# Nikhil-AI-Labs/image-super-resolution-2

Measured on AMD Instinct MI355X. Metric: output MPix/s at x4 SR (256->1024), higher is better.
Workload: dtype bf16 (bf16 MFMA operands, fp32 accumulate, fp32 activations in HBM); 1 GPU; FreqFusion x4 full 3-expert forward (HAT-L + DAT + NAFNet-SR + fusion stack), one 256x256 LR tile -> 1024x1024 per step per GPU (BASELINE configs[1]); seeded synthetic weights (172.3 M params), 1/f-noise tiles; tile=256, parallelism=tile-sharded x1, weights RCCL-broadcast once (0.0 ms), no per-tile collectives, launch=hipGraph replay, tiles_in_flight=2

## Files before the change

### image-super-resolution-2_amd/build.py

```python
from __future__ import annotations

import os
import subprocess
import sys
from concurrent.futures import ThreadPoolExecutor

HERE = os.path.dirname(os.path.abspath(__file__))
CSRC = os.path.join(HERE, "csrc")
LIB = os.path.join(HERE, "libff_hip.so")
SOURCES = ["ff_runtime.hip", "conv_gemm.hip", "conv_gemm_bf16.hip", "gemm_rows_bf16.hip", "conv3x3_halo.hip", "sgfn_tail.hip", "ocab_attn.hip", "conv3x3_small.hip", "attention.hip", "attention_bf16.hip", "win_attn_fused.hip", "hab_link.hip", "chan_qkv.hip", "token_mlp.hip", "token_linear.hip", "naf_fused.hip", "naf_tail.hip", "norm_pool.hip", "dwconv.hip", "elementwise.hip",
           "resample.hip", "freq.hip", "fusion_ops.hip", "metrics.hip", "train_ops.hip", "sr_losses.hip", "augment.hip", "ff_executor.hip"]
HIPCC = os.environ.get("HIPCC", "/opt/rocm/bin/hipcc")
FLAGS = ["--offload-arch=gfx950", "-O3", "-fPIC", "-std=c++17", "-Wall", "-Wno-unused-function", "-I" + os.path.join(HERE, "build")]


def _stale() -> bool:
    if not os.path.exists(LIB):
        return True
    t = os.path.getmtime(LIB)
    deps = [os.path.join(CSRC, f) for f in os.listdir(CSRC)] + [os.path.join(HERE, "..", "include", "ff_kernels.h")]
    return any(os.path.getmtime(d) > t for d in deps)


def gen_dispatch(path: str) -> None:
    from .lib import parse_header
    protos = {n: p for n, p in parse_header().items() if p[1] and p[1][-1] == "void*" and p[0] == "int"
              and n not in ("ff_forward", "ff_create", "ff_upload")}
    names = sorted(protos)
    out = ["// generated by build.py from include/ff_kernels.h -- do not edit", f"#define FF_DISPATCH_COUNT {len(names)}",
           "static const char* const FF_DISPATCH_NAMES[FF_DISPATCH_COUNT] = {" + ", ".join(f'"{n}"' for n in names) + "};"]
    def kinds(n):
        ks = []
        for i, ty in enumerate(protos[n][1]):
# ... 57 lines not shown
```

### image-super-resolution-2_amd/csrc/conv3x3_halo.hip

```cpp
#include "ff_common.h"

struct HaloParams {
  const float* in; const unsigned char* w; const float* bias; const float* mul; const float* res; float* out;
  int B, H, W, Cin, ldi, Cout, ldo, ldr, nchunk, tiles_x, tiles_y, nblk, act, shuffle;
  float alpha;
  float* pool_part;
  int vec_epi;
  int io_bf16;
  int images;
  FF_STAMP_MEMBER
};

#define HX_ROW 272
#define HX_W 18
#define HX_PROW 5120

template <int N> __device__ __forceinline__ void halo_wait_vmcnt() {
  static_assert(N >= 0 && N <= 12, "counted vmcnt out of range");
  if constexpr (N == 0) asm volatile("s_waitcnt vmcnt(0)" ::: "memory");
  else if constexpr (N == 1) asm volatile("s_waitcnt vmcnt(1)" ::: "memory");
  else if constexpr (N == 2) asm volatile("s_waitcnt vmcnt(2)" ::: "memory");
  else if constexpr (N == 3) asm volatile("s_waitcnt vmcnt(3)" ::: "memory");
  else if constexpr (N == 4) asm volatile("s_waitcnt vmcnt(4)" ::: "memory");
  else if constexpr (N == 5) asm volatile("s_waitcnt vmcnt(5)" ::: "memory");
// ... 206 lines not shown
            }
  #pragma unroll
            for (int i = 0; i < MI; ++i)
  #pragma unroll
              for (int j = 0; j < NI; ++j) {
                if (NTERMS == 3) {
                  acc[i][j] = __builtin_amdgcn_mfma_f32_32x32x16_bf16(ah[i], bl[j], acc[i][j], 0, 0, 0);
                  acc[i][j] = __builtin_amdgcn_mfma_f32_32x32x16_bf16(al[i], bh[j], acc[i][j], 0, 0, 0);
                }
                acc[i][j] = __builtin_amdgcn_mfma_f32_32x32x16_bf16(ah[i], bh[j], acc[i][j], 0, 0, 0);
              }
          }
        }
      }
      if (chunk + 1 < p.nchunk) {
        __syncthreads();
        if (!XPREF) load_x(chunk + 1);
        store_x();
      }
    }
  }
  FF_STAMP(8, 2);
  if (p.vec_epi) {
    asm volatile("s_waitcnt lgkmcnt(0)" ::: "memory");
    __builtin_amdgcn_s_barrier();
    float* ps = reinterpret_cast<float*>(smem);
    float* patch = reinterpret_cast<float*>(smem + 8192) + wid * (32 * 36);
    const int tq = lane >> 3, q4 = 4 * (lane & 7);
    const bool has_res = p.res != nullptr;
    constexpr bool RES_AHEAD = !(TWO_PER_CU || (NTERMS == 1 && MI * NI <= 2 && WM * WN == 4));
    f32x4 rq[2][MI][4];
    auto load_res = [&](int j, f32x4 (&dst)[MI][4]) {
#pragma unroll
      for (int i = 0; i < MI; ++i)
#pragma unroll
        for (int k = 0; k < 4; ++k) {
          const int mrow = tq + 8 * k, c4 = n0 + wc * TN + j * 32 + q4;
          const int oy = y0 + (wr * MI + i) * 2 + (mrow >> 4), ox = x0 + (mrow & 15);
          const bool ok = c4 < p.Cout && oy < p.H && ox < p.W;
          dst[i][k] = ok ? *reinterpret_cast<const f32x4*>(p.res + ((long long)(b * p.H + oy) * p.W + ox) * p.ldr + c4) : (f32x4){0.f, 0.f, 0.f, 0.f};
        }
    };
    if (RES_AHEAD && has_res) load_res(0, rq[0]);
#pragma unroll
    for (int j = 0; j < NI; ++j) {
      const int n = n0 + wc * TN + j * 32 + l31;
      const bool nok = n < p.Cout;
      const float bv = (nok && p.bias) ? p.bias[n] : 0.f;
      const float mv = ((nok && p.mul) ? p.mul[n] : 1.f) * p.alpha;
      const int c4 = n0 + wc * TN + j * 32 + q4;
      const bool cok = c4 < p.Cout;
      if (RES_AHEAD && has_res && j + 1 < NI) load_res(j + 1, rq[(j + 1) & 1]);
      f32x4 mv4 = {p.alpha, p.alpha, p.alpha, p.alpha};
      if (p.mul && cok) mv4 = *reinterpret_cast<const f32x4*>(p.mul + c4) * p.alpha;
      float psum = 0.f;
#pragma unroll
      for (int i = 0; i < MI; ++i) {
        const int ry0 = y0 + (wr * MI + i) * 2;
#pragma unroll
        for (int r = 0; r < 16; ++r) {
          const int mrow = (r & 3) + 8 * (r >> 2) + 4 * hh;
          const float a = ff_act_c<ACT, true>(acc[i][j][r] + bv);
          patch[mrow * 36 + l31] = a;
          if (nok && ry0 + (mrow >> 4) < p.H && x0 + (mrow & 15) < p.W) psum += a * mv;
        }
#pragma unroll
        for (int k = 0; k < 4; ++k) {
          const int mrow = tq + 8 * k;
          const int oy = ry0 + (mrow >> 4), ox = x0 + (mrow & 15);
          const bool ok = cok && oy < p.H && ox < p.W;
          const f32x4 a4 = *reinterpret_cast<const f32x4*>(patch + mrow * 36 + q4);
          const long long pix = ok ? ((long long)(b * p.H + oy) * p.W + ox) : 0;
          f32x4 r4 = {0.f, 0.f, 0.f, 0.f};
          if (RES_AHEAD && has_res) r4 = rq[j & 1][i][k];
          else if (has_res && ok) r4 = *reinterpret_cast<const f32x4*>(p.res + pix * p.ldr + c4);
          f32x4 v4;
#pragma unroll
          for (int e = 0; e < 4; ++e) v4[e] = __builtin_fmaf(a4[e], mv4[e], r4[e]);
          if (ok) {
            if (NTERMS == 1 && (p.io_bf16 & 2)) {
              bf16x4 h4;
#pragma unroll
              for (int e = 0; e < 4; ++e) h4[e] = (__bf16)v4[e];
              *reinterpret_cast<bf16x4*>(reinterpret_cast<__bf16*>(p.out) + pix * p.ldo + c4) = h4;
            } else {
              *reinterpret_cast<f32x4*>(p.out + pix * p.ldo + c4) = v4;
            }
          }
        }
      }
      if (p.pool_part) {
        psum += __shfl_xor(psum, 32);
        if (hh == 0) ps[wr * BN + wc * TN + j * 32 + l31] = psum;
      }
    }
    if (p.pool_part) {
      __syncthreads();
      for (int c = threadIdx.x; c < BN; c += NT) {
        float sacc = 0.f;
#pragma unroll
        for (int w = 0; w < WM; ++w) sacc += ps[w * BN + c];
        p.pool_part[(long long)blockIdx.x * BN + c] = sacc;
      }
    }
  } else
  {
    const bool has_res = p.res != nullptr;
#pragma unroll
    for (int j = 0; j < NI; ++j) {
      const int n = n0 + wc * TN + j * 32 + l31;
      const bool nok = n < p.Cout;
      const int nc = nok ? n : 0;
      const float bv = (nok && p.bias) ? p.bias[n] : 0.f;
      const float mv = ((nok && p.mul) ? p.mul[n] : 1.f) * p.alpha;
      float psum = 0.f;
#pragma unroll
      for (int i = 0; i < MI; ++i) {
        long long oidx[16];
        float rv[16];
        bool okp[16];
        const int ry0 = y0 + (wr * MI + i) * 2;
#pragma unroll
        for (int r = 0; r < 16; ++r) {
          const int mrow = (r & 3) + 8 * (r >> 2) + 4 * hh;
          const int oy = ry0 + (mrow >> 4), ox = x0 + (mrow & 15);
          okp[r] = nok && oy < p.H && ox < p.W;
          if (p.shuffle == 2) {
// ... 161 lines not shown
```

### image-super-resolution-2_amd/experts.py

```python
from __future__ import annotations

from typing import Dict, List, Optional

import torch

from . import ops
from .prep import (pack_conv, pack_dw, bn_scale_shift, fold_bn_after_conv, pack_token_linear, pack_naf_ffn, pack_naf_tail,
                   pack_win_attn, pack_win_rel, pack_token_projmlp, pack_chan_qkv, pack_token_linear_gated, pack_rel_overlap, pack_ocab_qkv)

T = torch.Tensor
SD = Dict[str, T]
RGB_MEAN = (0.4488, 0.4371, 0.4040)


def _ceil_to(n: int, m: int) -> int:
    return (n + m - 1) // m * m


class _Weights:

    def __init__(self, sd: SD, dev, prefix: str):
        self.sd, self.dev, self.p = sd, dev, prefix

    def __call__(self, name: str) -> T:
# ... 116 lines not shown
            self.gconv.append((w.conv(f"layers.{g}.conv"), w(f"layers.{g}.conv.bias")))

    def _mlp(self, x: T, blk: dict) -> T:
        xn = ops.layernorm(x, *blk["n2"])
        h = ops.linear(xn, *blk["fc1"], act="gelu")
        return ops.linear(h, *blk["fc2"], res=x)

    def hab(self, x: T, blk: dict) -> T:
        _, H, W, C = x.shape
        d = C // self.heads
        fused = ops.fused_modes()
        b16 = ops.gemm_mode() == "bf16" and H * W >= 1024 and C % 4 == 0
        att = ops.empty_rows_bf16(tuple(x.shape), x.device) if b16 else ops.empty_like_rows(x)
        s = blk["shift"]
        if fused:
            relp = _packed(blk, "relp", lambda: pack_win_rel(blk["rel"], self.ws, self.ws))
            _, xn = ops.win_attn_fused(x, att, _wf(blk, self.heads, d), relp, gamma=blk["n1"][0], beta=blk["n1"][1], H=H, W=W,
                                       Hp=H, Wp=W, win=(self.ws, self.ws), shift=(s, s), use_mask=s > 0, want_xn="bf16" if b16 else True)
        else:
            xn = ops.layernorm(x, *blk["n1"])
            qkv = ops.linear(xn, *blk["qkv"])
            ops.window_attn(qkv, att, blk["bias"], q_off=0, k_off=C, v_off=2 * C, o_off=0, H=H, W=W, Hp=H, Wp=W, win=(self.ws, self.ws),
                            kwin=(self.ws, self.ws), shift=(s, s), use_mask=s > 0, heads=self.heads, d=d, scale=d ** -0.5)
        c1 = ops.conv2d(xn, *blk["cab0"], ksize=(3, 3), pad=(1, 1), act="gelu", out_bf16=b16, per_image=True)
        c2, c2mean = ops.conv2d(c1, *blk["cab2"], ksize=(3, 3), pad=(1, 1), want_pool="partials", out_bf16=b16)
        gate = ops.vec_mlp(c2mean, *blk["ca1"], "relu", *blk["ca2"], "sigmoid", post=self.conv_scale)
        if fused:
            return ops.token_projmlp(att, x, _pm(blk), blk["n2"][0], blk["n2"][1], c2=c2, c2_scale=gate if x.shape[0] > 1 else gate.reshape(-1))
        t = ops.mix2(x, c2, cb=gate)
        x = ops.linear(att, *blk["proj"], res=t)
        return self._mlp(x, blk)

    def ocab_block(self, x: T, blk: dict) -> T:
        _, H, W, C = x.shape
        d = C // self.heads
        fused = ops.fused_modes()
        rows16 = ops.gemm_mode() == "bf16" and (self.ws, self.ows, d) == (16, 24, 30) and H % 16 == 0 and W % 16 == 0
        if rows16:
            pk = _packed(blk, "qkv_r16", lambda: pack_ocab_qkv(*blk["qkv"], self.heads, d))
            qkv = ops.token_linear_rows16(x, pk, gamma=blk["n1"][0], beta=blk["n1"][1])
        elif fused:
            qkv = ops.token_linear(x, _tl(blk, "qkv"), gamma=blk["n1"][0], beta=blk["n1"][1])
        else:
            qkv = ops.linear(ops.layernorm(x, *blk["n1"]), *blk["qkv"])
        if rows16:
            att = ops.empty_rows_bf16(tuple(x.shape), x.device)
            hp = self.heads * 32
            ops.ocab_attn_rows16(qkv, att, blk["rel"], q_off=0, k_off=hp, v_off=2 * hp, H=H, W=W, heads=self.heads, d=d, ws=self.ws,
                                 ows=self.ows)
        else:
            att = ops.empty_like_rows(x)
            ops.window_attn(qkv, att, blk["bias"], q_off=0, k_off=C, v_off=2 * C, o_off=0, H=H, W=W, Hp=H, Wp=W, win=(self.ws, self.ws),
                            kwin=(self.ows, self.ows), shift=(0, 0), use_mask=False, heads=self.heads, d=d, scale=d ** -0.5)
        if fused:
            return ops.token_projmlp(att, x, _pm(blk), blk["n2"][0], blk["n2"][1])
        x = ops.linear(att, *blk["proj"], res=x)
        return self._mlp(x, blk)

    def _linked(self, x: T) -> bool:
        B, H, W, C = x.shape
        return (ops.gemm_mode() == "bf16" and H * W >= 1024 and (self.ws, self.heads, C) == (16, 6, 180) and H % 16 == 0 and W % 16 == 0
                and B * H * W * 192 < 2 ** 31)

    def _habs_linked(self, x: T, blks: List[dict]) -> T:
        B, H, W, C = x.shape
        d, win = C // self.heads, (self.ws, self.ws)

        def relp(blk):
            return _packed(blk, "relp", lambda: pack_win_rel(blk["rel"], self.ws, self.ws))

        s = blks[0]["shift"]
        att = ops.empty_rows_bf16(tuple(x.shape), x.device)
        _, xn = ops.win_attn_fused(x, att, _wf(blks[0], self.heads, d), relp(blks[0]), gamma=blks[0]["n1"][0], beta=blks[0]["n1"][1], H=H, W=W,
                                   Hp=H, Wp=W, win=win, shift=(s, s), use_mask=s > 0, want_xn="bf16")
        for i, blk in enumerate(blks):
            c1 = ops.conv2d(xn, *blk["cab0"], ksize=(3, 3), pad=(1, 1), act="gelu", out_bf16=True, per_image=True)
            c2, c2mean = ops.conv2d(c1, *blk["cab2"], ksize=(3, 3), pad=(1, 1), want_pool="partials", out_bf16=True)
            gate = ops.vec_mlp(c2mean, *blk["ca1"], "relu", *blk["ca2"], "sigmoid", post=self.conv_scale)
            gate = gate if B > 1 else gate.reshape(-1)
            if i + 1 < len(blks):
                nxt = blks[i + 1]
                s = nxt["shift"]
                x, xn, att = ops.hab_link(att, x, _pm(blk), blk["n2"][0], blk["n2"][1], c2=c2, c2_scale=gate, wf=_wf(nxt, self.heads, d),
                                          rel_padded=relp(nxt), gamma1=nxt["n1"][0], beta1=nxt["n1"][1], shift=(s, s), use_mask=s > 0)
            else:
                x = ops.token_projmlp(att, x, _pm(blk), blk["n2"][0], blk["n2"][1], c2=c2, c2_scale=gate)
        return x

    def group(self, x: T, g: int) -> T:
        if self._linked(x):
            y = self._habs_linked(x, self.blocks[g])
        else:
            y = x
            for blk in self.blocks[g]:
                y = self.hab(y, blk)
        y = self.ocab_block(y, self.ocab[g])
        return ops.conv2d(y, *self.gconv[g], ksize=(3, 3), pad=(1, 1), res=x, per_image=True)

    def forward(self, lr: T, taps: Optional[dict] = None, feats: Optional[dict] = None, out: Optional[T] = None) -> T:
        B, _, h, w = lr.shape
# ... 351 lines not shown
```

### image-super-resolution-2_amd/ops.py

```python
from __future__ import annotations

from typing import Dict, Optional, Tuple

import torch

from . import lib as _lib

ACT = {None: 0, "none": 0, "gelu": 1, "relu": 2, "lrelu": 3, "sigmoid": 4}
T = torch.Tensor

_PROF = None
_META = [0.0, 0.0]


def _note(flops: float = 0.0, nbytes: float = 0.0):
    _META[0] += flops
    _META[1] += nbytes


def _numel(*ts) -> float:
    return float(sum(t.numel() * (t.element_size() / 4.0) for t in ts if t is not None))


def _instrument(fn):
# ... 686 lines not shown
    if tuple(c2_scale.shape) not in (((K,), (1, K)) if B == 1 else ((B, K),)) or not c2_scale.is_contiguous():
        raise _lib.FFError(f"hab_link: c2_scale must be [{K}] for one image or one row per image [{B},{K}], got {tuple(c2_scale.shape)}")
    if tuple(rel_padded.shape[:2]) != (wf["heads"], 31) or not rel_padded.is_contiguous():
        raise _lib.FFError("hab_link: rel_padded must be [heads][31][stride]")
    out = empty_like_rows(x)
    op_, ldo_, *_ = _nhwc(out, "hab_link.out")
    xn = empty_rows_bf16(tuple(x.shape), x.device)
    xnp, ldxn, *_ = _nhwc(xn, "hab_link.xn|bf16ok")
    ao = empty_rows_bf16(tuple(x.shape), x.device)
    aop, ldao, *_ = _nhwc(ao, "hab_link.att_out|bf16ok")
    m = pk["mlp"]
    _lib.check(_L().ff_hab_link(ap, lda, xp, ldx, cp, ldc, _ptr(c2_scale), K, B, H * W, op_, ldo_, B * H * W, K, m["ht"],
                                pk["proj"]["w"].data_ptr(), pk["proj"]["b"].data_ptr(), gamma2.data_ptr(), beta2.data_ptr(), float(eps2),
                                m["w"].data_ptr(), m["b1"].data_ptr(), m["b2"].data_ptr(), 1, 3,
                                aop, ldao, 0, gamma1.data_ptr(), beta1.data_ptr(), float(eps1), wf["w"].data_ptr(), wf["b"].data_ptr(),
                                rel_padded.data_ptr(), rel_padded.shape[1], rel_padded.shape[2], H, W, 16, 16, shift[0], shift[1],
                                int(use_mask), wf["heads"], wf["d"], xnp, ldxn, 1, 1, _stream()))
    rows, nwin, nh, d = B * H * W, B * (H // 16) * (W // 16), wf["heads"], wf["d"]
    _note(2.0 * rows * K * K + 4.0 * rows * K * m["ht"] * 32 + 2.0 * nwin * 256 * K * 3 * nh * d + 4.0 * nwin * nh * 256 * 256 * d,
          4.0 * rows * K * 3.0 + 4.0 * rows * (K * 0.5 + nh * d * 0.5))
    return out, xn, ao


def token_linear(x: T, pk: dict, *, gamma: Optional[T] = None, beta: Optional[T] = None, eps: float = 1e-5, act=None,
                 res: Optional[T] = None, res2: Optional[T] = None, res2_scale: Optional[T] = None, want_xn: bool = False,
                 stats_range: Optional[Tuple[int, int]] = None, stats_eps: float = 1e-5):
    xp, ldx, rows, K = rows_view(x, "token_linear.x")
    if K != pk["K"]:
        raise _lib.FFError("token_linear: K mismatch")
    N = pk["N"]
    out = empty_rows(tuple(x.shape[:-1]) + (N,), x.device)
    op, ldo, _, _ = rows_view(out, "token_linear.out")
    rp, ldr, r2p, ldr2 = None, 0, None, 0
    if res is not None:
        rp, ldr, rr, rc = rows_view(res, "token_linear.res")
        if rr != rows or rc != N:
            raise _lib.FFError("token_linear: res shape mismatch")
    if res2 is not None:
        r2p, ldr2, rr, rc = rows_view(res2, "token_linear.res2")
        if rr != rows or rc != N or res2_scale is None or res2_scale.numel() != N:
            raise _lib.FFError("token_linear: res2 shape mismatch")
    xn, xnp, ldxn = None, None, 0
    if want_xn:
        if gamma is None:
            raise _lib.FFError("token_linear: want_xn needs LayerNorm parameters")
        xn = empty_like_rows(x)
# ... 778 lines not shown
            _AA_TABLES.clear()
        span, wt = aa_tables(n_in, n_out)
        ent = _AA_TABLES[key] = (torch.from_numpy(span).to(device), torch.from_numpy(wt).to(device))
    return ent


def resize_aa(x: T, size: Tuple[int, int]) -> T:
    _chk(x, "resize_aa.x")
    if x.dim() != 4 or x.shape[1] != 3 or not x.is_contiguous() or x.numel() == 0:
        raise _lib.FFError("resize_aa: expected a non-empty contiguous [B,3,H,W] tensor")
    B, C, Hi, Wi = x.shape
    Ho, Wo = (int(v) for v in size)
    if Ho < 1 or Wo < 1 or Hi != 4 * Ho or Wi != 4 * Wo:
        raise _lib.FFError(f"resize_aa: only the x1/4 ratio is built: {Hi}x{Wi} -> {Ho}x{Wo} is refused")
    span_w, wt_w = _aa_tables_dev(Wi, Wo, x.device)
    span_h, wt_h = _aa_tables_dev(Hi, Ho, x.device)
    out = torch.empty((B, C, Ho, Wo), device=x.device, dtype=torch.float32)
    _lib.check(_L().ff_resize_aa(x.data_ptr(), out.data_ptr(), B * C, Hi, Wi, Ho, Wo, span_w.data_ptr(), wt_w.data_ptr(),
                                 span_h.data_ptr(), wt_h.data_ptr(), _stream()))
    _note(0.0, 4.0 * B * C * (Hi * Wi + Ho * Wo))
    return out


for _n in ("conv2d", "sgfn_tail", "ocab_attn", "ocab_attn_rows16", "token_linear_rows16", "linear", "win_attn_fused", "token_projmlp", "hab_link", "token_linear_gated", "token_mlp", "token_linear", "pixel_mlp", "dwconv3_gate_pool", "naf_front", "naf_ffn", "naf_tail", "window_attn", "layernorm", "pool_mean", "vec_mlp", "dwconv2d", "dwconv3x3_ln", "mix2", "fma3", "affine",
           "nchw_to_nhwc", "nhwc_to_nchw", "resize", "avgpool2", "dct8_bands", "dwt_pass", "fft_bands", "chan_attn_weights", "chan_qkv_attn",
           "band_mha_core", "band_weight", "freq_guidance", "dynamic_gates", "fuse_blend", "tile_accum", "tile_normalize"):
    globals()[_n] = _instrument(globals()[_n])
```

### include/ff_kernels.h

```cpp
#ifndef FF_KERNELS_H
#define FF_KERNELS_H
#ifdef __cplusplus
extern "C" {
#endif

#define FF_ACT_NONE 0
#define FF_ACT_GELU 1
#define FF_ACT_RELU 2
#define FF_ACT_LRELU 3
#define FF_ACT_SIGMOID 4

const char* ff_last_error(void);
int ff_abi_version(void);
int ff_device_cu_count(void);

int ff_conv2d(const float* in, const float* w, const float* bias, const float* mul, const float* res, float* out,
              int B, int H, int W, int Cin, int ldi, int Ho, int Wo, int Cout, int ldo, int ldr, int KH, int KW,
              int sy, int sx, int py, int px, int act, float alpha, int shuffle, int tile_hint, void* stream);

int ff_conv2d_bf16s(const float* in, const void* w_hi, const void* w_lo, int Kp, int Cp, const float* bias, const float* mul,
                    const float* res, float* out, int B, int H, int W, int Cin, int ldi, int Ho, int Wo, int Cout,
                    int ldo, int ldr, int KH, int KW, int sy, int sx, int py, int px, int act, float alpha, int shuffle,
                    int nterms, int tile_hint, const float* kmul, void* stream);
int ff_conv2d_bf16s_tile(long long M, int Cout, int K, int vec4);
// ... 46 lines not shown
int ff_hab_link(const float* att, int lda, const float* x, int ldx, const float* c2, int ldc, const float* c2_scale,
                int scale_ld, int B, long long rows_per_image, float* x_out, int ldxo, long long M, int K, int hidden_tiles,
                const void* proj_tiles, const float* proj_bias_padded, const float* gamma2, const float* beta2, float eps2,
                const void* mlp_tiles, const float* b1_padded, const float* b2, int nterms, int io_bf16,
                float* att_out, int ldo, int o_off, const float* gamma1, const float* beta1, float eps1,
                const void* qkv_tiles, const float* qkv_bias_padded, const float* rel_padded, int rel_rows, int rel_stride,
                int H, int W, int wh, int ww, int shift_h, int shift_w, int use_mask, int nheads, int d,
                float* xn_out, int ldxn, int out_bf16, int xn_bf16, void* stream);

int ff_token_mlp(const float* x, int ldx, float* out, int ldo, long long M, int K, int hidden_tiles, int N,
                 const float* gamma, const float* beta, float eps, const void* w_tiles, const float* b1_padded,
                 const float* b2, int nterms, void* stream);

long long ff_conv3x3_halo_weight_bytes(int Cout, int Cin, int bn, int nterms);
long long ff_conv3x3_halo_pool_rows(int B, int H, int W, int Cout, int bn, int nterms);
int ff_pool_finish(const float* part, int rows, int ld, int C, float inv_count, float* out, void* stream);
int ff_conv3x3_halo(const float* in, int ldi, const void* w_img, int bn, const float* bias, const float* mul,
                    const float* res, int ldr, float* out, int ldo, int B, int H, int W, int Cin, int Cout,
                    int act, float alpha, int shuffle, float* pool_partials, int nterms, int io_bf16, void* stream);
long long ff_conv3x3_halo_images_pool_rows(int B, int H, int W, int Cout, int bn, int nterms);
int ff_conv3x3_halo_images(const float* in, int ldi, const void* w_img, int bn, const float* bias, const float* mul,
                           const float* res, int ldr, float* out, int ldo, int B, int H, int W, int Cin, int Cout,
                           int act, float alpha, int shuffle, float* pool_partials, int nterms, int io_bf16, void* stream);

int ff_token_linear(const float* x, int ldx, float* out, int ldo, long long M, int K, int kpad, int N, int n_tiles,
                    const float* gamma, const float* beta, float eps, const void* w_tiles, const float* bias_padded,
                    int act, const float* res, int ldr, const float* res2, int ldr2, const float* res2_scale,
                    float* xn_out, int ldxn, float* stats_out, int stat_lo,
                    int stat_hi, float stat_eps, int nterms, void* stream);

int ff_token_linear_rows16(const float* x, int ldx, void* out16, int ldo, long long M, int K, int kpad, int N, int n_tiles,
                           const float* gamma, const float* beta, float eps, const void* w_tiles, const float* bias_padded,
                           const float* col_scale, int act, const float* res, int ldr, const float* res2, int ldr2,
                           const float* res2_scale, float* xn_out, int ldxn, float* stats_out, int stat_lo,
                           int stat_hi, float stat_eps, int nterms, void* stream);

int ff_token_linear_gated(const float* x, int ldx, const float* x2, int ldx2, const float* cm, const float* gw1t, const float* gb1,
                          const float* gw2, float gb2, float* out, int ldo, long long M, int K, int N, int n_tiles,
                          const void* w_tiles, const float* bias_padded, const float* res, int ldr, int nterms, void* stream);
int ff_token_linear_gated_images(const float* x, int ldx, const float* x2, int ldx2, const float* cm, int B, long long rows_per_image,
                                 const float* gb1, const float* gw2, float gb2, float* out, int ldo, long long M, int K, int N, int n_tiles,
                                 const void* w_tiles, const float* bias_padded, const float* res, int ldr, int nterms, void* stream);

long long ff_dwconv3_gate_pool_workspace(int C);
int ff_dwconv3_gate_pool(const float* in, int ldi, float* out, int ldo, int H, int W, int C, const float* w_tapmajor,
                         const float* bias, float* pooled, float* work, long long work_floats, void* stream);
// ... 229 lines not shown
```

Baseline: 27.56 output MPix/s.

## Fuse HAT CAB conv3x3-GELU-conv3x3 pair into one halo kernel

Adds a dedicated kernel that computes the CAB block's first 3x3 conv (180->60, GELU) on an 18x18 halo tile held in LDS and feeds it straight into the second 3x3 conv (60->180), which writes the pooled partials through the shared vector epilogue. This removes the intermediate c1 activation round-trip through HBM and one kernel launch per CAB. Both weight rings are streamed with async global-to-LDS loads, and the conv2 ring reuses the input-chunk space. The cost is recomputing the halo border for conv1, a single block per CU because of the large LDS footprint, and a kernel that only accepts the 180/60/180 bf16 shape. The existing halo epilogue is moved into an include file so both kernels share it.

```diff
diff --git a/image-super-resolution-2_amd/build.py b/image-super-resolution-2_amd/build.py
--- a/image-super-resolution-2_amd/build.py
+++ b/image-super-resolution-2_amd/build.py
@@ -8,7 +8,7 @@
 HERE = os.path.dirname(os.path.abspath(__file__))
 CSRC = os.path.join(HERE, "csrc")
 LIB = os.path.join(HERE, "libff_hip.so")
-SOURCES = ["ff_runtime.hip", "conv_gemm.hip", "conv_gemm_bf16.hip", "gemm_rows_bf16.hip", "conv3x3_halo.hip", "sgfn_tail.hip", "ocab_attn.hip", "conv3x3_small.hip", "attention.hip", "attention_bf16.hip", "win_attn_fused.hip", "hab_link.hip", "chan_qkv.hip", "token_mlp.hip", "token_linear.hip", "naf_fused.hip", "naf_tail.hip", "norm_pool.hip", "dwconv.hip", "elementwise.hip",
+SOURCES = ["ff_runtime.hip", "conv_gemm.hip", "conv_gemm_bf16.hip", "gemm_rows_bf16.hip", "conv3x3_halo.hip", "cab_fused.hip", "sgfn_tail.hip", "ocab_attn.hip", "conv3x3_small.hip", "attention.hip", "attention_bf16.hip", "win_attn_fused.hip", "hab_link.hip", "chan_qkv.hip", "token_mlp.hip", "token_linear.hip", "naf_fused.hip", "naf_tail.hip", "norm_pool.hip", "dwconv.hip", "elementwise.hip",
            "resample.hip", "freq.hip", "fusion_ops.hip", "metrics.hip", "train_ops.hip", "sr_losses.hip", "augment.hip", "ff_executor.hip"]
 HIPCC = os.environ.get("HIPCC", "/opt/rocm/bin/hipcc")
 FLAGS = ["--offload-arch=gfx950", "-O3", "-fPIC", "-std=c++17", "-Wall", "-Wno-unused-function", "-I" + os.path.join(HERE, "build")]
diff --git a/image-super-resolution-2_amd/csrc/cab_fused.hip b/image-super-resolution-2_amd/csrc/cab_fused.hip
--- /dev/null
+++ b/image-super-resolution-2_amd/csrc/cab_fused.hip
@@ -0,0 +1,283 @@
+#include "ff_common.h"
+
+extern "C" long long ff_conv3x3_halo_weight_bytes(int Cout, int Cin, int bn, int nterms);
+
+struct CabParams {
+  const __bf16* in; const unsigned char* w1; const unsigned char* w2; const float* bias1;
+  const float* bias; const float* mul; const float* res; float* out; float* pool_part;
+  int B, H, W, Cin, ldi, Cmid, Cout, ldo, ldr, tiles_x, tiles_y, io_bf16;
+  float alpha;
+  FF_STAMP_MEMBER
+};
+
+#define CAB_ROWB 144
+#define CAB_XPROW 3104
+#define CAB_CPROW 2816
+#define CAB_XBYTES (20 * CAB_XPROW)
+#define CAB_CBYTES (18 * CAB_CPROW)
+#define CAB_W1SLOT 9216
+#define CAB_W1SLOTS 5
+#define CAB_W2SLOT 15360
+#define CAB_W2SLOTS 4
+#define CAB_LDS (CAB_XBYTES + CAB_CBYTES + CAB_W1SLOTS * CAB_W1SLOT)
+static_assert(CAB_LDS <= 160 * 1024, "LDS budget");
+static_assert(CAB_W2SLOTS * CAB_W2SLOT <= CAB_XBYTES, "conv2's weight ring lives in the input chunk's space");
+static_assert(8192 + 8 * 32 * 36 * 4 <= CAB_XBYTES, "the epilogue's pool row and patches live in the input chunk's space");
+static_assert(CAB_XPROW % 16 == 0 && (CAB_XPROW / 4) % 64 == (18 * 36) % 64, "input rows continue the 36-dword pixel step across the row wrap");
+
+template <int N> __device__ __forceinline__ void cab_wait_vmcnt() {
+  static_assert(N >= 0 && N <= 63, "counted vmcnt out of range");
+  asm volatile("s_waitcnt vmcnt(%0)" ::"n"(N) : "memory");
+}
+template <int BEGIN, int END, class F> __device__ __forceinline__ void cab_static_for(F&& f) {
+  if constexpr (BEGIN < END) {
+    f(ff_ic<BEGIN>{});
+    cab_static_for<BEGIN + 1, END>(f);
+  }
+}
+
+__global__ __launch_bounds__(512, 1)
+void cab_fused_kernel(CabParams p) {
+  constexpr int WM = 4, WN = 2, MI = 2, NI = 3, NTERMS = 1, ACT = ACT_NONE;
+  constexpr int NW = WM * WN, NT = NW * 64, BN = WN * NI * 32, TN = NI * 32;
+  constexpr bool TWO_PER_CU = false;
+  constexpr int ROWB = CAB_ROWB, PROW = CAB_CPROW;
+  constexpr int W2ROW = 80, W1ROW = 144;
+  constexpr int NPX = 400, PPP = NT / 8, NPASS = (NPX + PPP - 1) / PPP;
+  constexpr int NQ = 324, MI1 = 3;
+  constexpr int NT1 = 27, DEPTH1 = CAB_W1SLOTS - 1, NT2 = 18, DEPTH2 = CAB_W2SLOTS - 1, XTAP = 4;
+  extern __shared__ __attribute__((aligned(16))) unsigned char smem[];
+  unsigned char* Xs = smem;
+  unsigned char* Cs = smem + CAB_XBYTES;
+  unsigned char* W1s = Cs + CAB_CBYTES;
+  unsigned char* W2s = smem;
+
+  const int tid = threadIdx.x, lane = tid & 63, wid = __builtin_amdgcn_readfirstlane(tid >> 6);
+  const int l31 = lane & 31, hh = lane >> 5;
+  const int wr = wid / WN, wc = wid % WN;
+  const int wm1 = wid >> 1, wn1 = wid & 1;
+  const bool third = wm1 < 3;
+
+  const int bpi = p.tiles_x * p.tiles_y;
+  const int b = (int)blockIdx.x / bpi;
+  const int L = ff_xcd_remap((int)blockIdx.x - b * bpi, bpi);
+  const int tx = L % p.tiles_x, ty = L / p.tiles_x;
+  const int y0 = ty * 16, x0 = tx * 16;
+  constexpr int n0 = 0;
+
+  auto dma1 = [&](int T, int slot) {
+    const unsigned char* src = p.w1 + (long long)T * CAB_W1SLOT + lane * 16;
+#pragma unroll
+    for (int i = 0; i < 2; ++i) {
+      const int pc = wid + NW * i;
+      if (pc < 9)
+        __builtin_amdgcn_global_load_lds((const __attribute__((address_space(1))) void*)(src + pc * 1024),
+                                         (__attribute__((address_space(3))) void*)(W1s + slot * CAB_W1SLOT + pc * 1024), 16, 0, 0);
+    }
+  };
+  auto dma2 = [&](int T, int slot) {
+    const unsigned char* src = p.w2 + (long long)T * CAB_W2SLOT + lane * 16;
+#pragma unroll
+    for (int i = 0; i < 2; ++i) {
+      const int pc = wid + NW * i;
+      if (pc < 15)
+        __builtin_amdgcn_global_load_lds((const __attribute__((address_space(1))) void*)(src + pc * 1024),
+                                         (__attribute__((address_space(3))) void*)(W2s + slot * CAB_W2SLOT + pc * 1024), 16, 0, 0);
+    }
+  };
+  FF_STAMP(8, 0);
+#pragma unroll
+  for (int d = 0; d < DEPTH1; ++d) dma1(d, d);
+
+  const int cg = (tid & 7) * 8, prow = tid >> 3;
+  int goff[NPASS];
+#pragma unroll
+  for (int j = 0; j < NPASS; ++j) {
+    const int hp = j * PPP + prow;
+    const int hy = hp / 20, hx = hp - hy * 20;
+    const int iy = y0 - 2 + hy, ix = x0 - 2 + hx;
+    const bool ok = hp < NPX && (unsigned)iy < (unsigned)p.H && (unsigned)ix < (unsigned)p.W;
+    goff[j] = ok ? ((b * p.H + iy) * p.W + ix) * p.ldi + cg : -1;
+  }
+  bf16x8 xr[NPASS];
+  auto load_x = [&](int chunk) {
+    const int c0 = chunk * 64;
+    const bool cok = c0 + cg < p.Cin;
+#pragma unroll
+    for (int j = 0; j < NPASS; ++j) {
+      const bool ok = cok && goff[j] >= 0;
+      xr[j] = *reinterpret_cast<const bf16x8*>(p.in + (ok ? goff[j] + c0 : 0));
+    }
+  };
+  auto store_x = [&](int chunk) {
+    const int c0 = chunk * 64;
+#pragma unroll
+    for (int j = 0; j < NPASS; ++j) {
+      const int hp = j * PPP + prow;
+      const bool ok = goff[j] >= 0;
+      bf16x8 v;
+#pragma unroll
+      for (int e = 0; e < 8; ++e) v[e] = (ok && c0 + cg + e < p.Cin) ? xr[j][e] : (__bf16)0.f;
+      if (hp < NPX) *reinterpret_cast<bf16x8*>(Xs + (hp / 20) * CAB_XPROW + (hp % 20) * ROWB + (tid & 7) * 16) = v;
+    }
+  };
+  load_x(0);
+  store_x(0);
+  FF_STAMP(8, 1);
+
+  f32x16 acc1[MI1];
+#pragma unroll
+  for (int i = 0; i < MI1; ++i)
+#pragma unroll
+    for (int r = 0; r < 16; ++r) acc1[i][r] = 0.f;
+  int aoff1[MI1];
+#pragma unroll
+  for (int i = 0; i < MI1; ++i) {
+    int q = (wm1 + 4 * i) * 32 + l31;
+    q = q < NQ ? q : NQ - 1;
+    aoff1[i] = (q / 18) * CAB_XPROW + (q % 18) * ROWB + 16 * hh;
+  }
+  const int boff1 = (wn1 * 32 + l31) * W1ROW + 16 * hh;
+
+  cab_static_for<0, NT1>([&](auto Tc) {
+    constexpr int T = decltype(Tc)::value, chunk = T / 9, tap = T - 9 * chunk;
+    constexpr bool more_x = chunk + 1 < 3;
+    constexpr int dy = tap / 3, dx = tap - 3 * dy;
+    constexpr int young = NT1 - 1 - T < DEPTH1 - 1 ? NT1 - 1 - T : DEPTH1 - 1;
+    constexpr int xl = (tap > XTAP && more_x) ? NPASS : 0;
+    if (wid == 0) cab_wait_vmcnt<young * 2 + xl>();
+    else cab_wait_vmcnt<young + xl>();
+    asm volatile("s_waitcnt lgkmcnt(0)" ::: "memory");
+    __builtin_amdgcn_s_barrier();
+    if (T + DEPTH1 < NT1) dma1(T + DEPTH1, (T + DEPTH1) % CAB_W1SLOTS);
+    if (tap == XTAP && more_x) {
+      asm volatile("" ::: "memory");
+      load_x(chunk + 1);
+      asm volatile("" ::: "memory");
+    }
+    const unsigned char* xa = Xs + dy * CAB_XPROW + dx * ROWB;
+    const unsigned char* wb = W1s + (T % CAB_W1SLOTS) * CAB_W1SLOT;
+    bf16x8 ah[4][MI1], bh[4];
+#pragma unroll
+    for (int s = 0; s < 4; ++s) {
+#pragma unroll
+      for (int i = 0; i < MI1; ++i) ah[s][i] = *reinterpret_cast<const bf16x8*>(xa + aoff1[i] + 32 * s);
+      bh[s] = *reinterpret_cast<const bf16x8*>(wb + boff1 + 32 * s);
+    }
+#pragma unroll
+    for (int s = 0; s < 4; ++s) {
+      acc1[0] = __builtin_amdgcn_mfma_f32_32x32x16_bf16(ah[s][0], bh[s], acc1[0], 0, 0, 0);
+      acc1[1] = __builtin_amdgcn_mfma_f32_32x32x16_bf16(ah[s][1], bh[s], acc1[1], 0, 0, 0);
+      acc1[2] = __builtin_amdgcn_mfma_f32_32x32x16_bf16(ah[s][2], bh[s], acc1[2], 0, 0, 0);
+    }
+    if (tap == 8 && more_x) {
+      asm volatile("s_waitcnt lgkmcnt(0)" ::: "memory");
+      __builtin_amdgcn_s_barrier();
+      store_x(chunk + 1);
+    }
+  });
+  FF_STAMP(8, 2);
+
+  asm volatile("s_waitcnt lgkmcnt(0)" ::: "memory");
+  __builtin_amdgcn_s_barrier();
+#pragma unroll
+  for (int d = 0; d < DEPTH2; ++d) dma2(d, d);
+  {
+    const int n = wn1 * 32 + l31;
+    const bool nok = n < p.Cmid;
+    const float bv = nok ? p.bias1[n] : 0.f;
+#pragma unroll
+    for (int i = 0; i < MI1; ++i) {
+      if (i == 2 && !third) continue;
+      const int q0 = (wm1 + 4 * i) * 32 + 4 * hh;
+#pragma unroll
+      for (int r = 0; r < 16; ++r) {
+        const int q = q0 + (r & 3) + 8 * (r >> 2);
+        const int cy = q / 18, cx = q - cy * 18;
+        const int iy = y0 - 1 + cy, ix = x0 - 1 + cx;
+        const bool in_img = (unsigned)iy < (unsigned)p.H && (unsigned)ix < (unsigned)p.W;
+        const float a = __builtin_fmaf(ff_act_c<ACT_GELU, true>(acc1[i][r] + bv), 1.0f, 0.f);
+        const __bf16 h = (nok && in_img) ? (__bf16)a : (__bf16)0.f;
+        if (q < NQ) *reinterpret_cast<__bf16*>(Cs + cy * PROW + cx * ROWB + n * 2) = h;
+      }
+    }
+  }
+  FF_STAMP(8, 3);
+
+  f32x16 acc[MI][NI];
+#pragma unroll
+  for (int i = 0; i < MI; ++i)
+#pragma unroll
+    for (int j = 0; j < NI; ++j)
+#pragma unroll
+      for (int r = 0; r < 16; ++r) acc[i][j][r] = 0.f;
+  int aoff[MI], boff[NI];
+#pragma unroll
+  for (int i = 0; i < MI; ++i) aoff[i] = ((wr * MI + i) * 2 + (l31 >> 4)) * PROW + (l31 & 15) * ROWB + 16 * hh;
+#pragma unroll
+  for (int j = 0; j < NI; ++j) boff[j] = (wc * TN + j * 32 + l31) * W2ROW + 16 * hh;
+  cab_static_for<0, NT2>([&](auto Tc) {
+    constexpr int T = decltype(Tc)::value, tap = T / 2, half = T & 1;
+    constexpr int dy = tap / 3, dx = tap - 3 * dy;
+    constexpr int young = NT2 - 1 - T < DEPTH2 - 1 ? NT2 - 1 - T : DEPTH2 - 1;
+    if (wid < 7) cab_wait_vmcnt<young * 2>();
+    else cab_wait_vmcnt<young>();
+    asm volatile("s_waitcnt lgkmcnt(0)" ::: "memory");
+    __builtin_amdgcn_s_barrier();
+    if (T + DEPTH2 < NT2) dma2(T + DEPTH2, (T + DEPTH2) % CAB_W2SLOTS);
+    const unsigned char* xa = Cs + dy * PROW + dx * ROWB;
+    const unsigned char* wb = W2s + (T % CAB_W2SLOTS) * CAB_W2SLOT;
+#pragma unroll
+    for (int s = 0; s < 2; ++s) {
+      bf16x8 ah[MI], bh[NI];
+#pragma unroll
+      for (int i = 0; i < MI; ++i) ah[i] = *reinterpret_cast<const bf16x8*>(xa + aoff[i] + 32 * (half * 2 + s));
+#pragma unroll
+      for (int j = 0; j < NI; ++j) bh[j] = *reinterpret_cast<const bf16x8*>(wb + boff[j] + 32 * s);
+#pragma unroll
+      for (int i = 0; i < MI; ++i)
+#pragma unroll
+        for (int j = 0; j < NI; ++j) acc[i][j] = __builtin_amdgcn_mfma_f32_32x32x16_bf16(ah[i], bh[j], acc[i][j], 0, 0, 0);
+    }
+  });
+  FF_STAMP(8, 4);
+  {
+#include "conv3x3_halo_vec_epilogue.inc"
+  }
+  FF_STAMP(8, 5);
+  FF_STAMP_DRAINED(8, 6);
+}
+
+extern "C" int ff_cab_fused(const void* xn, int ldi, const void* w1_img, long long w1_bytes, const float* bias1,
+                            const void* w2_img, long long w2_bytes, const float* bias2, void* c2, int ldo, float* pool_partials,
+                            int B, int H, int W, int Cin, int Cmid, int Cout, int nterms, int io_bf16, void* stream) {
+  FF_CHECK_ARG(nterms == 1, "ff_cab_fused: plain bf16 only (nterms must be 1)");
+  FF_CHECK_ARG(io_bf16 == 3, "ff_cab_fused: xn and c2 must be bf16 rows (io_bf16 == 3)");
+  FF_CHECK_ARG(Cin == 180 && Cmid == 60 && Cout == 180, "ff_cab_fused: built for 180 -> 60 -> 180 channels");
+  FF_CHECK_ARG(B > 0 && H > 0 && W > 0 && H % 16 == 0 && W % 16 == 0, "ff_cab_fused: H and W must be multiples of 16");
+  FF_CHECK_ARG((long long)H * W >= 1024, "ff_cab_fused: H * W must be at least 1024");
+  FF_CHECK_ARG(xn && w1_img && w2_img && bias1 && bias2 && c2 && pool_partials, "ff_cab_fused: null pointer");
+  FF_CHECK_ARG(ldi % 8 == 0 && ldi >= Cin && (((uintptr_t)xn) & 15) == 0, "ff_cab_fused: xn rows must be 16-byte aligned (pitch %% 8 == 0)");
+  FF_CHECK_ARG(ldo % 4 == 0 && ldo >= Cout && (((uintptr_t)c2) & 15) == 0, "ff_cab_fused: c2 rows must be 8-byte aligned (pitch %% 4 == 0) on a 16-byte aligned base");
+  FF_CHECK_ARG((((uintptr_t)w1_img) & 15) == 0 && (((uintptr_t)w2_img) & 15) == 0, "ff_cab_fused: weight images must be 16-byte aligned");
+  FF_CHECK_ARG(w1_bytes == ff_conv3x3_halo_weight_bytes(Cmid, Cin, 64, 1), "ff_cab_fused: conv1's weight image is not the bn 64 halo image of its shape");
+  FF_CHECK_ARG(w2_bytes == ff_conv3x3_halo_weight_bytes(Cout, Cmid, 192, 1), "ff_cab_fused: conv2's weight image is not the bn 192 halo image of its shape");
+  FF_CHECK_ARG((long long)B * H * W * ldi < (1LL << 31) && (long long)B * H * W * ldo < (1LL << 31), "ff_cab_fused: rows too large for 32-bit offsets (B * H * W * pitch >= 2^31)");
+  FF_CHECK_ARG(xn != c2, "ff_cab_fused: c2 must not alias xn");
+  CabParams p;
+  p.in = (const __bf16*)xn; p.w1 = (const unsigned char*)w1_img; p.w2 = (const unsigned char*)w2_img; p.bias1 = bias1;
+  p.bias = bias2; p.mul = nullptr; p.res = nullptr; p.out = (float*)c2; p.pool_part = pool_partials;
+  p.B = B; p.H = H; p.W = W; p.Cin = Cin; p.ldi = ldi; p.Cmid = Cmid; p.Cout = Cout; p.ldo = ldo; p.ldr = 0;
+  p.tiles_x = W / 16; p.tiles_y = H / 16; p.io_bf16 = io_bf16; p.alpha = 1.0f;
+  FF_STAMP_ARM(p);
+  static bool attr_set = false;
+  if (!attr_set) {
+    hipError_t e = hipFuncSetAttribute(reinterpret_cast<const void*>(&cab_fused_kernel), hipFuncAttributeMaxDynamicSharedMemorySize, (int)CAB_LDS);
+    if (e != hipSuccess) { ff_set_error("ff_cab_fused: cannot raise dynamic LDS to %d: %s", (int)CAB_LDS, hipGetErrorString(e)); return FF_ERR_LAUNCH; }
+    attr_set = true;
+  }
+  const long long nblocks = (long long)B * p.tiles_x * p.tiles_y;
+  hipLaunchKernelGGL(cab_fused_kernel, dim3((unsigned)nblocks), dim3(512), CAB_LDS, (hipStream_t)stream, p);
+  FF_LAUNCH_CHECK("ff_cab_fused");
+  return FF_OK;
+}
diff --git a/image-super-resolution-2_amd/csrc/conv3x3_halo.hip b/image-super-resolution-2_amd/csrc/conv3x3_halo.hip
--- a/image-super-resolution-2_amd/csrc/conv3x3_halo.hip
+++ b/image-super-resolution-2_amd/csrc/conv3x3_halo.hip
@@ -252,87 +252,7 @@
   }
   FF_STAMP(8, 2);
   if (p.vec_epi) {
-    asm volatile("s_waitcnt lgkmcnt(0)" ::: "memory");
-    __builtin_amdgcn_s_barrier();
-    float* ps = reinterpret_cast<float*>(smem);
-    float* patch = reinterpret_cast<float*>(smem + 8192) + wid * (32 * 36);
-    const int tq = lane >> 3, q4 = 4 * (lane & 7);
-    const bool has_res = p.res != nullptr;
-    constexpr bool RES_AHEAD = !(TWO_PER_CU || (NTERMS == 1 && MI * NI <= 2 && WM * WN == 4));
-    f32x4 rq[2][MI][4];
-    auto load_res = [&](int j, f32x4 (&dst)[MI][4]) {
-#pragma unroll
-      for (int i = 0; i < MI; ++i)
-#pragma unroll
-        for (int k = 0; k < 4; ++k) {
-          const int mrow = tq + 8 * k, c4 = n0 + wc * TN + j * 32 + q4;
-          const int oy = y0 + (wr * MI + i) * 2 + (mrow >> 4), ox = x0 + (mrow & 15);
-          const bool ok = c4 < p.Cout && oy < p.H && ox < p.W;
-          dst[i][k] = ok ? *reinterpret_cast<const f32x4*>(p.res + ((long long)(b * p.H + oy) * p.W + ox) * p.ldr + c4) : (f32x4){0.f, 0.f, 0.f, 0.f};
-        }
-    };
-    if (RES_AHEAD && has_res) load_res(0, rq[0]);
-#pragma unroll
-    for (int j = 0; j < NI; ++j) {
-      const int n = n0 + wc * TN + j * 32 + l31;
-      const bool nok = n < p.Cout;
-      const float bv = (nok && p.bias) ? p.bias[n] : 0.f;
-      const float mv = ((nok && p.mul) ? p.mul[n] : 1.f) * p.alpha;
-      const int c4 = n0 + wc * TN + j * 32 + q4;
-      const bool cok = c4 < p.Cout;
-      if (RES_AHEAD && has_res && j + 1 < NI) load_res(j + 1, rq[(j + 1) & 1]);
-      f32x4 mv4 = {p.alpha, p.alpha, p.alpha, p.alpha};
-      if (p.mul && cok) mv4 = *reinterpret_cast<const f32x4*>(p.mul + c4) * p.alpha;
-      float psum = 0.f;
-#pragma unroll
-      for (int i = 0; i < MI; ++i) {
-        const int ry0 = y0 + (wr * MI + i) * 2;
-#pragma unroll
-        for (int r = 0; r < 16; ++r) {
-          const int mrow = (r & 3) + 8 * (r >> 2) + 4 * hh;
-          const float a = ff_act_c<ACT, true>(acc[i][j][r] + bv);
-          patch[mrow * 36 + l31] = a;
-          if (nok && ry0 + (mrow >> 4) < p.H && x0 + (mrow & 15) < p.W) psum += a * mv;
-        }
-#pragma unroll
-        for (int k = 0; k < 4; ++k) {
-          const int mrow = tq + 8 * k;
-          const int oy = ry0 + (mrow >> 4), ox = x0 + (mrow & 15);
-          const bool ok = cok && oy < p.H && ox < p.W;
-          const f32x4 a4 = *reinterpret_cast<const f32x4*>(patch + mrow * 36 + q4);
-          const long long pix = ok ? ((long long)(b * p.H + oy) * p.W + ox) : 0;
-          f32x4 r4 = {0.f, 0.f, 0.f, 0.f};
-          if (RES_AHEAD && has_res) r4 = rq[j & 1][i][k];
-          else if (has_res && ok) r4 = *reinterpret_cast<const f32x4*>(p.res + pix * p.ldr + c4);
-          f32x4 v4;
-#pragma unroll
-          for (int e = 0; e < 4; ++e) v4[e] = __builtin_fmaf(a4[e], mv4[e], r4[e]);
-          if (ok) {
-            if (NTERMS == 1 && (p.io_bf16 & 2)) {
-              bf16x4 h4;
-#pragma unroll
-              for (int e = 0; e < 4; ++e) h4[e] = (__bf16)v4[e];
-              *reinterpret_cast<bf16x4*>(reinterpret_cast<__bf16*>(p.out) + pix * p.ldo + c4) = h4;
-            } else {
-              *reinterpret_cast<f32x4*>(p.out + pix * p.ldo + c4) = v4;
-            }
-          }
-        }
-      }
-      if (p.pool_part) {
-        psum += __shfl_xor(psum, 32);
-        if (hh == 0) ps[wr * BN + wc * TN + j * 32 + l31] = psum;
-      }
-    }
-    if (p.pool_part) {
-      __syncthreads();
-      for (int c = threadIdx.x; c < BN; c += NT) {
-        float sacc = 0.f;
-#pragma unroll
-        for (int w = 0; w < WM; ++w) sacc += ps[w * BN + c];
-        p.pool_part[(long long)blockIdx.x * BN + c] = sacc;
-      }
-    }
+#include "conv3x3_halo_vec_epilogue.inc"
   } else
   {
     const bool has_res = p.res != nullptr;
diff --git a/image-super-resolution-2_amd/csrc/conv3x3_halo_vec_epilogue.inc b/image-super-resolution-2_amd/csrc/conv3x3_halo_vec_epilogue.inc
--- /dev/null
+++ b/image-super-resolution-2_amd/csrc/conv3x3_halo_vec_epilogue.inc
@@ -0,0 +1,81 @@
+    asm volatile("s_waitcnt lgkmcnt(0)" ::: "memory");
+    __builtin_amdgcn_s_barrier();
+    float* ps = reinterpret_cast<float*>(smem);
+    float* patch = reinterpret_cast<float*>(smem + 8192) + wid * (32 * 36);
+    const int tq = lane >> 3, q4 = 4 * (lane & 7);
+    const bool has_res = p.res != nullptr;
+    constexpr bool RES_AHEAD = !(TWO_PER_CU || (NTERMS == 1 && MI * NI <= 2 && WM * WN == 4));
+    f32x4 rq[2][MI][4];
+    auto load_res = [&](int j, f32x4 (&dst)[MI][4]) {
+#pragma unroll
+      for (int i = 0; i < MI; ++i)
+#pragma unroll
+        for (int k = 0; k < 4; ++k) {
+          const int mrow = tq + 8 * k, c4 = n0 + wc * TN + j * 32 + q4;
+          const int oy = y0 + (wr * MI + i) * 2 + (mrow >> 4), ox = x0 + (mrow & 15);
+          const bool ok = c4 < p.Cout && oy < p.H && ox < p.W;
+          dst[i][k] = ok ? *reinterpret_cast<const f32x4*>(p.res + ((long long)(b * p.H + oy) * p.W + ox) * p.ldr + c4) : (f32x4){0.f, 0.f, 0.f, 0.f};
+        }
+    };
+    if (RES_AHEAD && has_res) load_res(0, rq[0]);
+#pragma unroll
+    for (int j = 0; j < NI; ++j) {
+      const int n = n0 + wc * TN + j * 32 + l31;
+      const bool nok = n < p.Cout;
+      const float bv = (nok && p.bias) ? p.bias[n] : 0.f;
+      const float mv = ((nok && p.mul) ? p.mul[n] : 1.f) * p.alpha;
+      const int c4 = n0 + wc * TN + j * 32 + q4;
+      const bool cok = c4 < p.Cout;
+      if (RES_AHEAD && has_res && j + 1 < NI) load_res(j + 1, rq[(j + 1) & 1]);
+      f32x4 mv4 = {p.alpha, p.alpha, p.alpha, p.alpha};
+      if (p.mul && cok) mv4 = *reinterpret_cast<const f32x4*>(p.mul + c4) * p.alpha;
+      float psum = 0.f;
+#pragma unroll
+      for (int i = 0; i < MI; ++i) {
+        const int ry0 = y0 + (wr * MI + i) * 2;
+#pragma unroll
+        for (int r = 0; r < 16; ++r) {
+          const int mrow = (r & 3) + 8 * (r >> 2) + 4 * hh;
+          const float a = ff_act_c<ACT, true>(acc[i][j][r] + bv);
+          patch[mrow * 36 + l31] = a;
+          if (nok && ry0 + (mrow >> 4) < p.H && x0 + (mrow & 15) < p.W) psum += a * mv;
+        }
+#pragma unroll
+        for (int k = 0; k < 4; ++k) {
+          const int mrow = tq + 8 * k;
+          const int oy = ry0 + (mrow >> 4), ox = x0 + (mrow & 15);
+          const bool ok = cok && oy < p.H && ox < p.W;
+          const f32x4 a4 = *reinterpret_cast<const f32x4*>(patch + mrow * 36 + q4);
+          const long long pix = ok ? ((long long)(b * p.H + oy) * p.W + ox) : 0;
+          f32x4 r4 = {0.f, 0.f, 0.f, 0.f};
+          if (RES_AHEAD && has_res) r4 = rq[j & 1][i][k];
+          else if (has_res && ok) r4 = *reinterpret_cast<const f32x4*>(p.res + pix * p.ldr + c4);
+          f32x4 v4;
+#pragma unroll
+          for (int e = 0; e < 4; ++e) v4[e] = __builtin_fmaf(a4[e], mv4[e], r4[e]);
+          if (ok) {
+            if (NTERMS == 1 && (p.io_bf16 & 2)) {
+              bf16x4 h4;
+#pragma unroll
+              for (int e = 0; e < 4; ++e) h4[e] = (__bf16)v4[e];
+              *reinterpret_cast<bf16x4*>(reinterpret_cast<__bf16*>(p.out) + pix * p.ldo + c4) = h4;
+            } else {
+              *reinterpret_cast<f32x4*>(p.out + pix * p.ldo + c4) = v4;
+            }
+          }
+        }
+      }
+      if (p.pool_part) {
+        psum += __shfl_xor(psum, 32);
+        if (hh == 0) ps[wr * BN + wc * TN + j * 32 + l31] = psum;
+      }
+    }
+    if (p.pool_part) {
+      __syncthreads();
+      for (int c = threadIdx.x; c < BN; c += NT) {
+        float sacc = 0.f;
+#pragma unroll
+        for (int w = 0; w < WM; ++w) sacc += ps[w * BN + c];
+        p.pool_part[(long long)blockIdx.x * BN + c] = sacc;
+      }
+    }
diff --git a/image-super-resolution-2_amd/experts.py b/image-super-resolution-2_amd/experts.py
--- a/image-super-resolution-2_amd/experts.py
+++ b/image-super-resolution-2_amd/experts.py
@@ -162,8 +162,11 @@
             qkv = ops.linear(xn, *blk["qkv"])
             ops.window_attn(qkv, att, blk["bias"], q_off=0, k_off=C, v_off=2 * C, o_off=0, H=H, W=W, Hp=H, Wp=W, win=(self.ws, self.ws),
                             kwin=(self.ws, self.ws), shift=(s, s), use_mask=s > 0, heads=self.heads, d=d, scale=d ** -0.5)
-        c1 = ops.conv2d(xn, *blk["cab0"], ksize=(3, 3), pad=(1, 1), act="gelu", out_bf16=b16, per_image=True)
-        c2, c2mean = ops.conv2d(c1, *blk["cab2"], ksize=(3, 3), pad=(1, 1), want_pool="partials", out_bf16=b16)
+        if b16 and self._cab_fused(xn):
+            c2, c2mean = ops.cab_fused(xn, blk["cab0"], blk["cab2"])
+        else:
+            c1 = ops.conv2d(xn, *blk["cab0"], ksize=(3, 3), pad=(1, 1), act="gelu", out_bf16=b16, per_image=True)
+            c2, c2mean = ops.conv2d(c1, *blk["cab2"], ksize=(3, 3), pad=(1, 1), want_pool="partials", out_bf16=b16)
         gate = ops.vec_mlp(c2mean, *blk["ca1"], "relu", *blk["ca2"], "sigmoid", post=self.conv_scale)
         if fused:
             return ops.token_projmlp(att, x, _pm(blk), blk["n2"][0], blk["n2"][1], c2=c2, c2_scale=gate if x.shape[0] > 1 else gate.reshape(-1))
@@ -197,6 +200,9 @@
         x = ops.linear(att, *blk["proj"], res=x)
         return self._mlp(x, blk)
 
+    def _cab_fused(self, xn: T) -> bool:
+        return ops.cab_fused_ok(xn)
+
     def _linked(self, x: T) -> bool:
         B, H, W, C = x.shape
         return (ops.gemm_mode() == "bf16" and H * W >= 1024 and (self.ws, self.heads, C) == (16, 6, 180) and H % 16 == 0 and W % 16 == 0
@@ -214,8 +220,11 @@
         _, xn = ops.win_attn_fused(x, att, _wf(blks[0], self.heads, d), relp(blks[0]), gamma=blks[0]["n1"][0], beta=blks[0]["n1"][1], H=H, W=W,
                                    Hp=H, Wp=W, win=win, shift=(s, s), use_mask=s > 0, want_xn="bf16")
         for i, blk in enumerate(blks):
-            c1 = ops.conv2d(xn, *blk["cab0"], ksize=(3, 3), pad=(1, 1), act="gelu", out_bf16=True, per_image=True)
-            c2, c2mean = ops.conv2d(c1, *blk["cab2"], ksize=(3, 3), pad=(1, 1), want_pool="partials", out_bf16=True)
+            if self._cab_fused(xn):
+                c2, c2mean = ops.cab_fused(xn, blk["cab0"], blk["cab2"])
+            else:
+                c1 = ops.conv2d(xn, *blk["cab0"], ksize=(3, 3), pad=(1, 1), act="gelu", out_bf16=True, per_image=True)
+                c2, c2mean = ops.conv2d(c1, *blk["cab2"], ksize=(3, 3), pad=(1, 1), want_pool="partials", out_bf16=True)
             gate = ops.vec_mlp(c2mean, *blk["ca1"], "relu", *blk["ca2"], "sigmoid", post=self.conv_scale)
             gate = gate if B > 1 else gate.reshape(-1)
             if i + 1 < len(blks):
diff --git a/image-super-resolution-2_amd/ops.py b/image-super-resolution-2_amd/ops.py
--- a/image-super-resolution-2_amd/ops.py
+++ b/image-super-resolution-2_amd/ops.py
@@ -732,6 +732,49 @@
     return out, xn, ao
 
 
+def cab_fused_ok(x: T) -> bool:
+    if not isinstance(x, torch.Tensor) or x.dim() != 4 or x.dtype != torch.bfloat16 or not x.is_cuda:
+        return False
+    B, H, W, C = x.shape
+    if not (_HALO and _GEMM_MODE == "bf16" and C == 180 and H * W >= 1024 and H % 16 == 0 and W % 16 == 0):
+        return False
+    ld = x.stride(2)
+    rows_ok = x.stride(3) == 1 and x.stride(1) == W * ld and (B == 1 or x.stride(0) == H * W * ld)
+    return rows_ok and ld % 8 == 0 and ld >= C and x.data_ptr() % 16 == 0 and B * H * W * max(ld, 192) < 2 ** 31
+
+
+def cab_fused(xn: T, cab0: Tuple[T, T], cab2: Tuple[T, T], out: Optional[T] = None):
+    if _GEMM_MODE != "bf16":
+        raise _lib.FFError("cab_fused exists for the plain-bf16 contraction mode only")
+    if xn.dtype != torch.bfloat16:
+        raise _lib.FFError("cab_fused: xn must be bf16 rows")
+    from . import prep as _prep
+    xp, ldi, B, H, W, Cin = _nhwc(xn, "cab_fused.xn|bf16ok")
+    (w0, b0), (w2, b2) = cab0, cab2
+    Cmid, Cout = w0.shape[0], w2.shape[0]
+    if w0.dim() != 2 or w0.shape[1] != 9 * Cin or w2.dim() != 2 or w2.shape[1] != 9 * Cmid or b0 is None or b2 is None:
+        raise _lib.FFError(f"cab_fused: packed weights must be [Cmid, {9 * Cin}] and [Cout, 9 * Cmid], both with a bias")
+    img0 = PREPARED.get(w0, "halo1", lambda: (_prep.pack_conv3x3_halo(w0, Cin, _prep.halo_bn(Cmid), 1), _prep.halo_bn(Cmid)))
+    img2 = PREPARED.get(w2, "halo1", lambda: (_prep.pack_conv3x3_halo(w2, Cmid, _prep.halo_bn(Cout), 1), _prep.halo_bn(Cout)))
+    if (img0[1], img2[1]) != (64, 192):
+        raise _lib.FFError(f"cab_fused: weight images of tile widths {img0[1]} / {img2[1]}, built for 64 / 192")
+    oshape = (B, H, W, Cout)
+    if out is None:
+        out = empty_rows_bf16(oshape, xn.device)
+    elif tuple(out.shape) != oshape or out.dtype != torch.bfloat16:
+        raise _lib.FFError(f"cab_fused: out must be bf16 rows {oshape}")
+    op, ldo, *_ = _nhwc(out, "cab_fused.out|bf16ok")
+    prow = int(_L().ff_conv3x3_halo_images_pool_rows(B, H, W, Cout, 192, 1))
+    if prow < 0:
+        raise _lib.FFError("cab_fused: bad shape")
+    part = torch.empty((prow, 192), device=xn.device, dtype=torch.float32)
+    _lib.check(_L().ff_cab_fused(xp, ldi, img0[0].data_ptr(), img0[0].numel() * img0[0].element_size(), _ptr(b0),
+                                 img2[0].data_ptr(), img2[0].numel() * img2[0].element_size(), _ptr(b2), op, ldo, part.data_ptr(),
+                                 B, H, W, Cin, Cmid, Cout, 1, 3, _stream()))
+    _note(2.0 * B * H * W * 9 * (Cin * Cmid + Cmid * Cout), 2.0 * _numel(xn, out) + 2.0 * _numel(w0, w2))
+    return out, PoolPartials(part, Cout, 1.0 / float(H * W), images=B)
+
+
 def token_linear(x: T, pk: dict, *, gamma: Optional[T] = None, beta: Optional[T] = None, eps: float = 1e-5, act=None,
                  res: Optional[T] = None, res2: Optional[T] = None, res2_scale: Optional[T] = None, want_xn: bool = False,
                  stats_range: Optional[Tuple[int, int]] = None, stats_eps: float = 1e-5):
@@ -1556,7 +1599,7 @@
     return out
 
 
-for _n in ("conv2d", "sgfn_tail", "ocab_attn", "ocab_attn_rows16", "token_linear_rows16", "linear", "win_attn_fused", "token_projmlp", "hab_link", "token_linear_gated", "token_mlp", "token_linear", "pixel_mlp", "dwconv3_gate_pool", "naf_front", "naf_ffn", "naf_tail", "window_attn", "layernorm", "pool_mean", "vec_mlp", "dwconv2d", "dwconv3x3_ln", "mix2", "fma3", "affine",
+for _n in ("conv2d", "cab_fused", "sgfn_tail", "ocab_attn", "ocab_attn_rows16", "token_linear_rows16", "linear", "win_attn_fused", "token_projmlp", "hab_link", "token_linear_gated", "token_mlp", "token_linear", "pixel_mlp", "dwconv3_gate_pool", "naf_front", "naf_ffn", "naf_tail", "window_attn", "layernorm", "pool_mean", "vec_mlp", "dwconv2d", "dwconv3x3_ln", "mix2", "fma3", "affine",
            "nchw_to_nhwc", "nhwc_to_nchw", "resize", "avgpool2", "dct8_bands", "dwt_pass", "fft_bands", "chan_attn_weights", "chan_qkv_attn",
            "band_mha_core", "band_weight", "freq_guidance", "dynamic_gates", "fuse_blend", "tile_accum", "tile_normalize"):
     globals()[_n] = _instrument(globals()[_n])
diff --git a/include/ff_kernels.h b/include/ff_kernels.h
--- a/include/ff_kernels.h
+++ b/include/ff_kernels.h
@@ -92,6 +92,10 @@
 int ff_conv3x3_halo_images(const float* in, int ldi, const void* w_img, int bn, const float* bias, const float* mul,
                            const float* res, int ldr, float* out, int ldo, int B, int H, int W, int Cin, int Cout,
                            int act, float alpha, int shuffle, float* pool_partials, int nterms, int io_bf16, void* stream);
+
+int ff_cab_fused(const void* xn, int ldi, const void* w1_img, long long w1_bytes, const float* bias1,
+                 const void* w2_img, long long w2_bytes, const float* bias2, void* c2, int ldo, float* pool_partials,
+                 int B, int H, int W, int Cin, int Cmid, int Cout, int nterms, int io_bf16, void* stream);
 
 int ff_token_linear(const float* x, int ldx, float* out, int ldo, long long M, int K, int kpad, int N, int n_tiles,
                     const float* gamma, const float* beta, float eps, const void* w_tiles, const float* bias_padded,
```

New measurement: 28.09 output MPix/s, median of 6. 1.02x the previous value.
